# mfkiwl/conan-slam

Measured on AMD Instinct MI355X. Metric: ekf_update_steps_per_sec, higher is better.
Workload: dtype f32

## Files before the change

conan_slam_amd/_capi.py:

```python
from __future__ import annotations

import ctypes as C
import os
import re

_HERE = os.path.dirname(os.path.abspath(__file__))
LIB_PATH = os.path.join(_HERE, "lib", "libcslam_hip.so")
HEADER_PATH = os.path.join(_HERE, "..", "include", "cslam.h")

OK, ERR_BAD_ARG, ERR_CAPACITY, ERR_HIP, ERR_NO_DEVICE, ERR_ALLOC = 0, 1, 2, 3, 4, 5
FACTOR_OK, FACTOR_FALLBACK, FACTOR_ZEROED, FACTOR_SKIPPED, FACTOR_BAD_IDF, FACTOR_INTERNAL = 0, 1, 2, 4, 8, 16
FACTOR_HEADING_SKIPPED = 32
F32, F64 = 0, 1
Q_LOWER_CHOL_GAIN, Q_PREDICT_NM4, Q_REF_EXACT, Q_TEXTBOOK = 1, 2, 3, 0
STAGE_GATHER, STAGE_FACTOR, STAGE_GAIN, STAGE_DOWNDATE, N_STAGES = 0, 1, 2, 3, 4
STAGE_NAMES = ["gather", "factor", "gain", "downdate"]


class CslamError(RuntimeError):
    def __init__(self, code: int, msg: str):
        super().__init__(f"cslam status {code}: {msg}")
        self.code = code


BATCH_MC_SYMBOLS = ("cslam_ekf_batch_predict_each", "cslam_ekf_batch_get_poses")

LANDMARK_SYMBOLS = ("cslam_ekf_get_landmarks", "cslam_ekf_batch_get_landmarks")
_PROTOTYPES = {
    "cslam_ekf_get_landmarks": [C.c_void_p, C.c_int, C.c_int, C.c_void_p, C.c_void_p, C.c_void_p],
    "cslam_ekf_batch_get_landmarks": [C.c_void_p, C.c_int, C.c_int, C.c_void_p, C.c_void_p, C.c_void_p],
    "cslam_ekf_rows_launches": [C.c_void_p, C.POINTER(C.c_longlong)],
    "cslam_ekf_pgemm_split": [C.c_void_p, C.POINTER(C.c_int), C.POINTER(C.c_int)],
    "cslam_ekf_batch_pgemm_split": [C.c_void_p, C.POINTER(C.c_int), C.POINTER(C.c_int)],
    "cslam_sim_batch_create": [C.c_void_p, C.c_int, C.c_int, C.POINTER(C.c_longlong), C.c_int, C.POINTER(C.c_void_p)],
    "cslam_sim_batch_destroy": [C.c_void_p],
    "cslam_sim_batch_scan": [C.c_void_p, C.c_void_p, C.c_double, C.c_void_p, C.c_longlong, C.POINTER(C.c_int),
                             C.POINTER(C.c_int), C.POINTER(C.c_int)],
    "cslam_sim_batch_get_scan": [C.c_void_p, C.c_int, C.c_void_p, C.c_void_p, C.c_void_p, C.c_void_p],
    "cslam_sim_batch_get_table": [C.c_void_p, C.c_void_p],
    "cslam_sim_batch_set_table": [C.c_void_p, C.c_void_p],
    "cslam_ekf_batch_update_scan": [C.c_void_p, C.c_void_p, C.c_void_p],
    "cslam_ekf_batch_augment_scan": [C.c_void_p, C.c_void_p, C.c_void_p],
    "cslam_pf_best_particle": [C.c_void_p, C.c_int, C.POINTER(C.c_int)] + [C.c_void_p] * 5,
    "cslam_pf_estimate": [C.c_void_p, C.POINTER(C.c_double), C.POINTER(C.c_double)] + [C.c_void_p] * 4,
    "cslam_pf_get_all_features": [C.c_void_p, C.c_void_p],
    "cslam_pf_best_particle_sharded": [C.c_void_p, C.c_void_p, C.c_int, C.POINTER(C.c_longlong)] + [C.c_void_p] * 5,
    "cslam_pf_estimate_sharded": [C.c_void_p, C.c_void_p, C.POINTER(C.c_double), C.POINTER(C.c_double)]
                                 + [C.c_void_p] * 4,
}
PF_ESTIMATE_SYMBOLS = tuple(k for k in _PROTOTYPES if k.startswith("cslam_pf_"))
PF_PICK_MAX, PF_PICK_MIN = 0, 1
SIM_BATCH_SYMBOLS = tuple(k for k in _PROTOTYPES if "sim_batch" in k or k.endswith("_scan"))

SCORE_FIELD_NAMES = ("POSE_N", "POSE_BAD", "POSE_IN", "POSE_ERR2", "POSE_EPHI2", "POSE_NEES",
                     "LM_N", "LM_BAD", "LM_IN", "LM_ERR2", "LM_NEES")
(SCORE_POSE_N, SCORE_POSE_BAD, SCORE_POSE_IN, SCORE_POSE_ERR2, SCORE_POSE_EPHI2, SCORE_POSE_NEES,
 SCORE_LM_N, SCORE_LM_BAD, SCORE_LM_IN, SCORE_LM_ERR2, SCORE_LM_NEES) = range(len(SCORE_FIELD_NAMES))
SCORE_FIELDS = len(SCORE_FIELD_NAMES)
_PROTOTYPES.update({
    "cslam_ekf_batch_score_reset": [C.c_void_p, C.c_int, C.c_double, C.c_double],
    "cslam_ekf_batch_score_set_truth": [C.c_void_p, C.c_void_p, C.c_int],
    "cslam_ekf_batch_score": [C.c_void_p, C.c_void_p],
    "cslam_ekf_batch_score_scan": [C.c_void_p, C.c_void_p, C.c_void_p],
    "cslam_ekf_batch_get_scores": [C.c_void_p, C.c_void_p, C.c_void_p, C.c_int, C.POINTER(C.c_int),
# ... 181 lines not shown
```

conan_slam_amd/csrc/cslam_ekf.hip:

```cpp
#include <hip/hip_runtime.h>

#include <algorithm>
#include <atomic>
#include <cfloat>
#include <cmath>
#include <cstdint>
#include <cstdlib>
#include <new>
#include <string>
#include <thread>
#include <vector>

#include "cslam_common.hpp"
#include "device_owners.hpp"
#include "ekf_kernels.hpp"
#include "ekf_kernels_fast.hpp"
#include "ekf_assoc_deferred_kernels.hpp"
#include "ekf_augment_kernels.hpp"
#include "ekf_counted_kernels.hpp"
#include "ekf_landmark_kernels.hpp"
#include "ekf_lookahead.hpp"
#include "ekf_options.hpp"
#include "ekf_pending_store.hpp"
#include "ekf_pgemm_limbs.hpp"
#include "ekf_pgemm_tiles.hpp"
#include "ekf_pose_kernels.hpp"
#define CSLAM_SCORE_SINGLE_ONLY
#include "ekf_score_kernels.hpp"
#include "ekf_staging.hpp"
#include "host_linalg.hpp"
#include "pf_host_parts.hpp"

namespace cslam
{
__global__ void ekf_la_signal_kernel(unsigned* signal, unsigned add)
{
    if (threadIdx.x == 0)
    {
        atomicAdd(signal, add);
    }
}
__device__ __forceinline__ bool la_wide_snapshot(const LaSnapJob& j)
{
    if (j.Z == nullptr || blockIdx.x + 1 != gridDim.x)
    {
        return false;
    }
    for (int i = threadIdx.x; i < 3 * j.m; i += 128)
    {
        if (i < 2 * j.m)
        {
            j.Z_out[i] = j.Z[i];
        }
        else
        {
            j.idf_out[i - 2 * j.m] = j.idf[i - 2 * j.m];
        }
    }
    return true;
}
__global__ void __launch_bounds__(128) ekf_la_wide_f32(LaWideArgs a)
{
    if (la_wide_snapshot(a.snap))
    {
        return;
    }
    ekf_la_wide_body<1, 0>(a);
}
__global__ void __launch_bounds__(128) ekf_la_wide_f32_k64(LaWideArgs a)
{
    if (la_wide_snapshot(a.snap))
    {
        return;
    }
    ekf_la_wide_body<1, 64>(a);
}

__global__ void __launch_bounds__(128) ekf_la_wide_f32_k64m(LaWideArgs a, float* WT)
{
    if (la_wide_snapshot(a.snap))
    {
        return;
    }
    ekf_la_wide_body<1, 64, 1>(a, WT);
}

__global__ void __launch_bounds__(256) ekf_la_blocks_mirror_kernel(LaPrepArgs<float> a, LaMirrorArgs mi)
{
    ekf_la_blocks_mirror_body(a, mi);
}
}

using namespace cslam;

namespace
{

std::atomic<int>& g_engines = ::cslam::live_engines();

constexpr size_t kLdsBudget    = 150 * 1024;

struct EkfBase
{
    explicit EkfBase(const EkfOptions& o) : opt(o) {}
    virtual ~EkfBase() {}
    const EkfOptions opt;
    int         dtype    = CSLAM_F32;
    int         device   = 0;
    int         quirks   = CSLAM_Q_REF_EXACT;
    int         nmax     = 0;
    int         ncap     = 0;
    int         ldp      = 0;
    int         n        = 3;
    int         sync_mode = 1;
    int         pgemm_wgs     = 0;
    int         split_whole = 0, split_strips = 0;
    Stream      stream_own, stream_b_own, stream_f_own;
    hipStream_t stream   = nullptr;
    hipStream_t stream_b = nullptr;
    long long   la_windows = 0;
    long long   stage_launches = 0;
    long long   rows_launches = 0;
    long long   augment_launches = 0;

    virtual int init()                                                                        = 0;
    virtual int set_state(const void* X, int n, const void* P, int ldp)                        = 0;
    virtual int get_state(void* X, void* P, int ldp)                                           = 0;
    virtual int get_x(void* X, int cap)                                                        = 0;
    virtual int get_landmarks(int first, int count, void* x, void* pll, void* pvl)             = 0;
    virtual int trace(double* tr)                                                              = 0;
    virtual int get_pose(void* x, void* pvv)                                                   = 0;
    virtual int score_reset(int series_capacity, double gate_pose, double gate_lm)             = 0;
    virtual int score_set_truth(const double* lm_true, int count)                              = 0;
    virtual int score(const double* xv_true, int with_map)                                     = 0;
    virtual int get_scores(double* totals, float* series, double* track, int capacity_records, int* records,
                           long long* calls)                                                   = 0;
    virtual int predict(double v, double swa, const void* Q, double wb, double dt)             = 0;
    virtual int update(const void* Z, int m, const void* R, const int* idf, int batch, bool on_device) = 0;
    virtual int augment(const void* Z, int q, const void* R)                                   = 0;
    virtual int augment_device(const void* dZ, int q, const void* R)                           = 0;
    virtual int observe_heading(double phi, int use)                                           = 0;
    virtual int associate(const void* Z, int m, const void* R, double g1, double g2, int* idf_out, int* kind) = 0;
    virtual int update_counted(const void* dZ, int m_cap, const void* R, const int* d_idf, const int* d_count,
                               int batch)                                                      = 0;
    virtual int associate_deferred(const void* Z, int m, const void* R, double g1, double g2, int* idf_out, int* kind,
                                   int* counts)                                                = 0;
    virtual int associate_deferred_async(const void* Z, int m, const void* R, double g1, double g2) = 0;
    virtual int association_wait(int* idf_out, int* kind, int* counts)                         = 0;
    virtual int association_device_ptrs(const void** dZF, const int** d_idf, const void** dZN,
                                        const int** d_counts)                                  = 0;
    virtual int factor_status(int* flags, int clear)                                           = 0;
    virtual int set_profiling(int on)                                                          = 0;
    virtual int get_stage_times(double* ms, int* launches)                                     = 0;
    virtual int debug_last_update(void* PHT, void* S, void* G, void* W1, void* V, int* k)      = 0;
    virtual int set_deferred(int max_cols)                                                     = 0;
// ... 1639 lines not shown
                return rc;
            }
        }
        CSLAM_HIP_TRY(hipStreamSynchronize(stream));
        return CSLAM_OK;
    }


    struct LaUpd
    {
        const T*       dZ;
        const int*     dIdf;
        int            m;
        T              R[4];
        PredictArgs<T> pp;
    };
    struct FactorOut
    {
        DevBuf<T>   S, G, Gt, V, t, U, M, sub, xloc;
        DevBuf<int> idloc;
    };
    struct LaSet
    {
        Event          ev_fb;
        Event          ev_raw;
        FactorOut      fo[2];
        DevBuf<T>      XL, PvL, PH, PvLb, Dbb;
        DevBuf<T>      Y;
        DevBuf<LaModel<T>> model;
        DevBuf<unsigned>   done;
        DevBuf<long long>  stamps;
        DevBuf<int>        idf_keep;
        DevBuf<T>          z_keep;
    };
    struct LaHeld
    {
        bool       valid = false;
        bool       k64   = false;
        unsigned   grid  = 0;
        LaWideArgs wa;
        float*     wt = nullptr;
    };
    LaHeld      la_held;
    LaUpd       la_q[2];
    int         la_n = 0;
    LaSet       la;
    bool        la_ready = false;
    hipStream_t stream_f = nullptr;
    DevBuf<T>   la_WR;
    int         la_kpad  = 0;
    int         la_cus = 0;
    unsigned    la_target = 0;
    unsigned    la_seq    = 0;
    unsigned    la_sig_add = 0;
    DevBuf<float> la_WT;
    int           la_wt_rows     = 0;
    const T *dbgS = nullptr, *dbgGt = nullptr, *dbgV = nullptr;

    int la_ensure(int kp_cols)
    {
        constexpr int KM = 2 * kLaMaxObs;
        if (!la_ready)
        {
            int lo = 0, hi = 0;
            CSLAM_HIP_TRY(hipDeviceGetStreamPriorityRange(&lo, &hi));
            Stream sf;
            LaSet  nl;
            int    rc = sf.create_with_priority(hipStreamNonBlocking, hi);
            if (rc || (rc = nl.ev_fb.create(hipEventDisableTiming)) || (rc = nl.ev_raw.create(hipEventDisableTiming)))
            {
                return rc;
            }
            CSLAM_HIP_TRY(hipFuncSetAttribute(reinterpret_cast<const void*>(&ekf_la_chain_kernel<T, 32>),
                                              hipFuncAttributeMaxDynamicSharedMemorySize, (int)la_chain_lds<T>(32)));
            CSLAM_HIP_TRY(hipFuncSetAttribute(reinterpret_cast<const void*>(&ekf_la_chain_kernel<T, 64>),
                                              hipFuncAttributeMaxDynamicSharedMemorySize, (int)la_chain_lds<T>(64)));
            CSLAM_TRY(nl.done.alloc_zeroed_blocking(768));
            for (FactorOut& f : nl.fo)
            {
                const size_t kk = (size_t)KM * (KM + 1);
                if ((rc = f.S.alloc(kk)) || (rc = f.G.alloc(kk)) || (rc = f.Gt.alloc(kk)) || (rc = f.V.alloc(KM)) ||
                    (rc = f.t.alloc(KM)) || (rc = f.U.alloc(KM)) || (rc = f.M.alloc((size_t)3 * KM)) ||
                    (rc = f.sub.alloc((size_t)(3 + KM) * KM)) || (rc = f.xloc.alloc(3 + KM)) ||
                    (rc = f.idloc.alloc(kLaMaxObs)))
                {
                    return rc;
                }
            }
            if ((rc = nl.XL.alloc((size_t)2 * KM)) || (rc = nl.PvL.alloc((size_t)2 * KM * 3)) ||
                (rc = nl.PH.alloc((size_t)KM * KM)) || (rc = nl.PvLb.alloc((size_t)KM * 3)) ||
                (rc = nl.Dbb.alloc((size_t)KM * KM)) || (rc = nl.Y.alloc((size_t)KM * KM)) ||
                (rc = nl.model.alloc(2)) || (rc = nl.idf_keep.alloc(kLaMaxObs)) ||
                (rc = nl.z_keep.alloc(2 * kLaMaxObs)) ||
                (opt.la_stamps && (rc = nl.stamps.alloc_zeroed_blocking(32))))
            {
                return rc;
            }
            stream_f_own = std::move(sf);
            stream_f     = stream_f_own.get();
            la           = std::move(nl);
            la_cus       = 1;
            la_target    = 0;
            la_seq       = 0;
            la_ready     = true;
        }
        if (kp_cols > la_kpad)
        {
            CSLAM_HIP_TRY(hipStreamSynchronize(stream));
            CSLAM_HIP_TRY(hipStreamSynchronize(stream_f));
// ... 21 lines not shown
    {
        const int k = 2 * m;
        const bool on = opt.lookahead > 0 || (opt.lookahead < 0 && sizeof(T) == 4 && n >= 7000 && g_engines.load() == 1);
        return on && !sync_mode && !opt.pipeline && prof.mode != 1 && k > 16 && k <= 2 * kLaMaxObs && opt.gather_corr_wide &&
               opt.fuse_predict && (sizeof(T) == 4 || opt.fuse_f64) && defer_max >= k + (la_n ? 2 * la_q[0].m : k) &&
               pend.wcap >= k + (la_n ? 2 * la_q[0].m : k) && seq.count == 0 && pend.hd_cols[0] == 0 && pend.hd_cols[1] == 0 && n > 3 &&
               kp_call_limit == 0;
    }

    int la_launch_held_wide(const LaSnapJob* job)
    {
        if (!la_held.valid)
        {
            return CSLAM_OK;
        }
        if constexpr (std::is_same<T, float>::value)
        {
            int rc = use_device();
            if (rc)
            {
                return rc;
            }
            if (g_engines.load() > 1)
            {
                CSLAM_HIP_TRY(hipStreamWaitEvent(stream, la.ev_fb.get(), 0));
            }
            LaWideArgs& wa = la_held.wa;
            unsigned    g  = la_held.grid;
            if (job != nullptr)
            {
                wa.snap = *job;
                g += 1;
            }
            if (la_held.k64 && la_held.wt != nullptr)
            {
                hipLaunchKernelGGL(ekf_la_wide_f32_k64m, dim3(g), dim3(128), 0, stream, wa, la_held.wt);
            }
            else if (la_held.k64)
            {
                hipLaunchKernelGGL(ekf_la_wide_f32_k64, dim3(g), dim3(128), 0, stream, wa);
            }
            else
            {
                hipLaunchKernelGGL(ekf_la_wide_f32, dim3(g), dim3(128), 0, stream, wa);
            }
            CSLAM_HIP_TRY(hipGetLastError());
        }
        la_held.valid = false;
        return CSLAM_OK;
    }

    int la_enqueue(const T* dZ, const int* dIdf, int m, const T* R, bool on_device)
    {
        if (on_device && la_n == 0)
        {
            int rc = la_held.valid ? ensure_m(m) : CSLAM_OK;
            if (rc)
            {
                return rc;
            }
            if constexpr (std::is_same<T, float>::value)
            {
                if (la_held.valid)
                {
                    unsigned char* ds = ring.dev_slot(ring.take_slot());
                    LaSnapJob      job;
                    job.Z       = dZ;
// ... 264 lines not shown

    int la_launch_window(bool may_hold = false)
    {
        if (la_n == 0)
        {
            return CSLAM_OK;
        }
        const int   nu = la_n;
        const LaUpd ua = la_q[0], ub = la_q[nu - 1];
        const int   ka = 2 * ua.m, kb = nu == 2 ? 2 * ub.m : 0;
        la_n = 0;
        const PredictArgs<T> held = pp;
        int rc = use_device();
        if (rc)
        {
            return rc;
        }
        if (pend.kp > 256 && (rc = flush()))
        {
            return rc;
        }
        if ((rc = ensure_k(2 * kLaMaxObs)) || (rc = ensure_w(ka + kb)) || (rc = la_ensure(pend.kp)))
        {
            return rc;
        }
        if (opt.lower && (rc = ensure_tile_list(round_up(n, kTile) / kTile)))
        {
            return rc;
        }
        const bool safe = g_engines.load() > 1;
        const unsigned n_blocks = (unsigned)(3 + ka + 2 * kb);
        const bool hold = may_hold && opt.la_hold_wide && opt.la_fused && !safe && nu == 2 && std::is_same<T, float>::value &&
                 !la.stamps.get();
        auto launch_chain = [&]() -> int {
            const LaChainArgs<T> ch = la_chain_args(ua, ub, nu, hold, la_target + n_blocks, ++la_seq);
            if (std::max(ka, kb) <= 32)
            {
                hipLaunchKernelGGL((ekf_la_chain_kernel<T, 32>), dim3(1), dim3(256), la_chain_lds<T>(32), stream_f, ch);
            }
            else
            {
                hipLaunchKernelGGL((ekf_la_chain_kernel<T, 64>), dim3(1), dim3(256), la_chain_lds<T>(64), stream_f, ch);
            }
            CSLAM_HIP_TRY(hipGetLastError());
            CSLAM_HIP_TRY(hipEventRecord(la.ev_fb.get(), stream_f));
            return CSLAM_OK;
        };
        if (!safe && (rc = launch_chain()))
        {
            return rc;
        }
        bool use_mirror = false;
        if constexpr (std::is_same<T, float>::value)
        {
            use_mirror = opt.la_mirror &&
                         (pend.kp == 0 || (pend.mirror_covers(pend.kp, n) && pend.kp <= 128 && pend.kp % 4 == 0));
        }
        const int  k8f       = round_up(pend.kp, 8);
        const bool pg_signal = !opt.la_wg_signal && !safe && pend.kp > 0 && seq.count == 0 && sizeof(T) == 4 && k8f <= 128 &&
                               opt.lower && ldp < 32768 && !limbs_take(k8f) && stream_b == stream &&
                               pend.hd_cols[pend.wcur] == 0;
        if constexpr (std::is_same<T, float>::value)
        {
            if (use_mirror)
            {
                hipLaunchKernelGGL(ekf_la_blocks_mirror_kernel, dim3(n_blocks), dim3(256), 0, stream,
                                   la_prep_args(ua, ub, nu, hold, pg_signal), la_mirror_args(ua, ub, nu, hold));
            }
// ... 6 lines not shown
        }
        CSLAM_HIP_TRY(hipGetLastError());
        if (safe)
        {
            CSLAM_HIP_TRY(hipEventRecord(la.ev_raw.get(), stream));
            CSLAM_HIP_TRY(hipStreamWaitEvent(stream_f, la.ev_raw.get(), 0));
            if ((rc = launch_chain()))
            {
                return rc;
            }
        }
        la_target += n_blocks;
        la_sig_add = pg_signal ? n_blocks : 0u;
        rc         = flush();
        if (la_sig_add != 0)
        {
            const unsigned add = la_sig_add;
            la_sig_add         = 0;
            hipLaunchKernelGGL(ekf_la_signal_kernel, dim3(1), dim3(64), 0, stream, la.done.get(), add);
        }
        if (rc)
        {
            return rc;
        }
        bool fused = false;
        if constexpr (std::is_same<T, float>::value)
        {
            if (opt.la_fused)
            {
                fused = true;
                la_held.wa  = la_wide_args(ua, ub, nu, hold);
                la_held.k64 = opt.la_k64 && ua.m == 32 && ub.m == 32;
                la_held.wt = (opt.la_mirror && la_held.k64 && pend.kp == 0) ? la_WT.get() : nullptr;
                pend.mirror_written(la_held.wt ? ka + kb : 0, n);
                la_held.grid  = (unsigned)(round_up(n, kTile) / 32);
                la_held.valid = true;
                if (!hold && (rc = la_launch_held_wide(nullptr)))
                {
                    return rc;
                }
                last_slot = nullptr;
                last_k    = 0;
                pend.appended(ka + kb);
                sub_valid = false;
            }
        }
        if (!fused && ((rc = la_wide(ua, la.fo[0], la.ev_fb.get())) || (nu == 2 && (rc = la_wide(ub, la.fo[1], nullptr)))))
        {
            return rc;
        }
        pp = held;
        la_windows++;
        return (la.stamps.get() && la_windows == 300) ? la_report_stamps() : CSLAM_OK;
    }

    int la_report_stamps()
    {
        long long h[32];
        CSLAM_HIP_TRY(hipStreamSynchronize(stream));
        CSLAM_HIP_TRY(hipMemcpy(h, la.stamps.get(), sizeof(h), hipMemcpyDeviceToHost));
        fprintf(stderr, "[cslam la wide stamps, 10 ns ticks] ids+columns issue:%lld poll+DMA wait:%lld pht_a:%lld gain_a:%lld store+share W1_a:%lld pht_b+corr:%lld share+G_b:%lld gain_b:%lld store_b:%lld\n",
                h[17] - h[16], h[18] - h[17], h[19] - h[18], h[20] - h[19], h[21] - h[20], h[22] - h[21], h[23] - h[22],
                h[24] - h[23], h[25] - h[24]);
        fprintf(stderr, "[cslam la stamps, cycles] load+observe:%lld sums:%lld symmetrise:%lld cholesky:%lld (first half %lld) inverse:%lld outputs:%lld total:%lld\n",
                h[6] - h[0], h[7] - h[6], h[1] - h[7], h[2] - h[1], h[5] ? h[5] - h[1] : 0, h[3] - h[2], h[4] - h[3], h[4] - h[0]);
        return CSLAM_OK;
// ... 983 lines not shown
{
    CSLAM_NEED(h);
    if (!whole_tiles || !strips)
    {
        return fail(CSLAM_ERR_BAD_ARG, "pgemm_split: null");
    }
    *whole_tiles = B(h)->split_whole;
    *strips      = B(h)->split_strips;
    return CSLAM_OK;
}

int cslam_ekf_lookahead_windows(cslam_ekf_t h, long long* windows)
{
    CSLAM_NEED(h);
    if (!windows)
    {
        return fail(CSLAM_ERR_BAD_ARG, "lookahead_windows: null");
    }
    *windows = B(h)->la_windows;
    return CSLAM_OK;
}

int cslam_ekf_rows_launches(cslam_ekf_t h, long long* launches)
{
    CSLAM_NEED(h);
    if (!launches)
    {
        return fail(CSLAM_ERR_BAD_ARG, "rows_launches: null");
    }
    *launches = B(h)->rows_launches;
    return CSLAM_OK;
}

int cslam_ekf_stage_launches(cslam_ekf_t h, long long* launches)
{
    CSLAM_NEED(h);
    if (!launches)
    {
        return fail(CSLAM_ERR_BAD_ARG, "stage_launches: null");
    }
    *launches = B(h)->stage_launches;
    return CSLAM_OK;
}

int cslam_ekf_get_streams(cslam_ekf_t h, void** chain_stream, void** pgemm_stream)
{
    CSLAM_NEED(h);
    if (chain_stream)
    {
        *chain_stream = reinterpret_cast<void*>(B(h)->stream);
    }
    if (pgemm_stream)
    {
        *pgemm_stream = reinterpret_cast<void*>(B(h)->stream_b);
    }
    return CSLAM_OK;
}

int cslam_ekf_run_many(cslam_ekf_t* handles, int count, int steps, const double* v, const double* swa, const void* Q,
                       double wb, double dt, const void* const* dZ, const int* const* d_idf, int m, const void* R,
                       int batch)
{
    if (!handles || count < 0 || steps < 0 || m < 0 || !R || !Q || (steps > 0 && (!v || !swa)) || (m > 0 && (!dZ || !d_idf)))
    {
        return fail(CSLAM_ERR_BAD_ARG, "run_many: bad arguments");
    }
// ... 99 lines not shown
```

conan_slam_amd/csrc/ekf_lookahead.hpp:

```cpp
#pragma once

#include <hip/hip_runtime.h>

#include "ekf_kernels.hpp"
#include "ekf_kernels_fast.hpp"

namespace cslam
{

constexpr int kLaMaxObs = 32;

__device__ inline int la_row(const int* __restrict__ idf, int s, int n)
{
    return 3 + 2 * clamp_idf(idf[s >> 1], n) - 2 + (s & 1);
}

template <typename T>
struct LaRowsArgs
{
    const T* X;
    const T* Pv;
    int      ldp, n;
    const int* idf_a;
    int        ra;
// ... 903 lines not shown
        mo.g02 = s_g[0];
        mo.g12 = s_g[1];
    }
    if (tid < 3)
    {
        mo.pose[tid] = xl[tid];
    }
    if (tid < 9)
    {
        mo.pvv[tid] = s_pvv[tid];
    }
    for (int e = tid; e < mb * 10; e += 256)
    {
        mo.coef[e] = coef[e];
    }
}

constexpr int kFlagLaTimeout = 16;

template <typename T>
struct LaChainArgs
{
    FactorArgs<T>   fa, fb;
    T *             du_a, *du_b;
    LaCarryArgs<T>  ca;
    int             nu;
    const unsigned* done;
    unsigned        target;
    unsigned long long timeout;
    unsigned*       chain_done;
    unsigned        seq;
};

template <typename T, int K>
__device__ __forceinline__ void ekf_la_chain_body(const LaChainArgs<T>& a)
{
    extern __shared__ __align__(16) unsigned char la_chain_smem[];
    if (threadIdx.x < 64)
    {
        const unsigned long long t0 = __builtin_amdgcn_s_memrealtime();
        while (true)
        {
            unsigned c = threadIdx.x < 16
                             ? __hip_atomic_load(a.done + 16 * threadIdx.x, __ATOMIC_RELAXED, __HIP_MEMORY_SCOPE_AGENT)
                             : 0u;
            c += __shfl_xor(c, 1);
            c += __shfl_xor(c, 2);
            c += __shfl_xor(c, 4);
            c += __shfl_xor(c, 8);
            c = __shfl(c, 0);
            if ((int)(c - a.target) >= 0)
            {
                break;
            }
            __builtin_amdgcn_s_sleep(32);
            if (__builtin_amdgcn_s_memrealtime() - t0 > a.timeout)
            {
                if (threadIdx.x == 0)
                {
                    atomicOr(&a.fa.flags[0], kFlagLaTimeout);
                }
                break;
            }
        }
    }
    __syncthreads();
    __builtin_amdgcn_fence(__ATOMIC_ACQUIRE, "agent");
    if constexpr (std::is_same<T, float>::value)
    {
        ekf_factor_mfma_f32_body<K>(a.fa, a.du_a);
    }
    else
    {
        ekf_factor_mfma_f64_body<K>(a.fa, a.du_a);
    }
    if (a.nu == 2)
    {
        __builtin_amdgcn_fence(__ATOMIC_RELEASE, "workgroup");
        __syncthreads();
        __builtin_amdgcn_fence(__ATOMIC_ACQUIRE, "workgroup");
        ekf_la_carry_body<T>(a.ca, la_chain_smem);
        __builtin_amdgcn_fence(__ATOMIC_RELEASE, "workgroup");
        __syncthreads();
        __builtin_amdgcn_fence(__ATOMIC_ACQUIRE, "workgroup");
        if constexpr (std::is_same<T, float>::value)
        {
            ekf_factor_mfma_f32_body<K>(a.fb, a.du_b);
        }
        else
        {
            ekf_factor_mfma_f64_body<K>(a.fb, a.du_b);
        }
    }
    __builtin_amdgcn_fence(__ATOMIC_RELEASE, "agent");
    __syncthreads();
    if (threadIdx.x < 32)
    {
        __hip_atomic_store(a.chain_done + 16 * threadIdx.x, a.seq, __ATOMIC_RELAXED, __HIP_MEMORY_SCOPE_AGENT);
    }
}

template <typename T, int K>
__global__ void __launch_bounds__(256) ekf_la_chain_kernel(LaChainArgs<T> a)
{
    ekf_la_chain_body<T, K>(a);
}

struct LaSnapJob
{
    const float* Z;
    const int*   idf;
    float*       Z_out;
    int*         idf_out;
    int          m;
};

struct LaWideArgs
{
    const float* P;
    int          ldp, n, lower;
    float*       X;
    float*       Pv;
    int          nu;
    const int *  idf_a, *idf_b;
    int          ma, mb;
    int          valid_a, valid_b, w_a, w_b;
// ... 620 lines not shown
```

conan_slam_amd/csrc/ekf_options.hpp:

```cpp
#pragma once

#include <algorithm>
#include <cstdlib>
#include <cstring>

namespace cslam
{
inline int env_int(const char* name, int dflt) { const char* s = getenv(name); return s ? atoi(s) : dflt; }
inline int env_flag(const char* name, int dflt) { const char* s = getenv(name); return s ? (atoi(s) ? 1 : 0) : dflt; }
constexpr int kPgemmTailMax = 1 << 20;
inline int env_pgemm_tail(int dflt) { return std::max(-1, std::min(kPgemmTailMax, env_int("CSLAM_PGEMM_TAIL", dflt))); }

struct EkfOptions
{
    int fuse_predict = 1;
    int fuse_f64     = 1;
    int seq_defer    = 1;
    int lower = 1;
    int pipeline    = 0;
    int pgemm_spare = 16;
    int gather_corr_wide = 1;
    int lookahead    = -1;
    int la_hold_wide = 1;
    int la_k64       = 1;
    int la_wg_signal = 0;
    int la_mirror    = 1;
    int la_fused     = 1;
    int la_stamps    = 0;
    int pgemm_limbs = 0;
    int limbs_kmin  = 65;
    int xcd_queues = 0;
    int psym_nt    = -1;
    int pgemm_tail = -1;
    int f64_kcm = 16;
    int f64_cb  = 0;

    static EkfOptions from_env()
    {
        EkfOptions o;
        o.fuse_predict     = env_int("CSLAM_FUSE_PREDICT", o.fuse_predict);
        o.fuse_f64         = env_flag("CSLAM_FUSE_F64", o.fuse_f64);
        o.seq_defer        = env_int("CSLAM_SEQ_DEFER", o.seq_defer);
        const char* sv     = getenv("CSLAM_STORAGE");
        o.lower            = (sv && !strcmp(sv, "full")) ? 0 : 1;
        o.pipeline         = env_flag("CSLAM_PIPELINE", o.pipeline);
        o.pgemm_spare      = std::max(0, env_int("CSLAM_PGEMM_SPARE", o.pgemm_spare));
        o.gather_corr_wide = env_flag("CSLAM_GATHER_WIDE", o.gather_corr_wide);
        const int la       = env_int("CSLAM_LOOKAHEAD", o.lookahead);
        o.lookahead        = la > 0 ? 1 : (la < 0 ? -1 : 0);
        o.la_hold_wide     = env_flag("CSLAM_LA_HOLD_WIDE", o.la_hold_wide);
        o.la_k64           = env_flag("CSLAM_LA_K64", o.la_k64);
        o.la_wg_signal     = env_flag("CSLAM_LA_WG_SIGNAL", o.la_wg_signal);
        o.la_mirror        = env_flag("CSLAM_LA_MIRROR", o.la_mirror);
        o.la_fused         = env_flag("CSLAM_LA_FUSED", o.la_fused);
        o.la_stamps        = getenv("CSLAM_LA_STAMPS") ? 1 : 0;
        const int limbs    = env_int("CSLAM_PGEMM_LIMBS", o.pgemm_limbs);
        o.pgemm_limbs      = (limbs == 6 || limbs == 9) ? limbs : 0;
        const int kmin     = env_int("CSLAM_LIMBS_KMIN", o.limbs_kmin);
        o.limbs_kmin       = kmin < 0 ? o.limbs_kmin : std::max(57, kmin);
        o.xcd_queues       = env_flag("CSLAM_XCD_QUEUES", o.xcd_queues);
        o.psym_nt          = env_flag("CSLAM_PSYM_NT", o.psym_nt);
        o.pgemm_tail       = env_pgemm_tail(o.pgemm_tail);
        o.f64_kcm          = std::max(4, std::min(64, (env_int("CSLAM_F64_KCM", o.f64_kcm) + 3) / 4 * 4));
        if (getenv("CSLAM_F64_CB"))
        {
            o.f64_cb = env_int("CSLAM_F64_CB", 0) == 2 ? 2 : 4;
        }
        return o;
    }
};

struct EkfBatchOptions
{
    int wg_signal  = 0;
    int wide_pairs = 2;
    int la_k64     = 1;
    int stamps     = 0;
    int pgemm_tail = -1;

    static EkfBatchOptions from_env()
    {
        EkfBatchOptions o;
        o.wg_signal  = env_flag("CSLAM_BATCH_WG_SIGNAL", o.wg_signal);
        o.wide_pairs = env_int("CSLAM_BATCH_WIDE_PAIRS", o.wide_pairs) == 1 ? 1 : 2;
        o.la_k64     = env_flag("CSLAM_LA_K64", o.la_k64);
        o.stamps     = getenv("CSLAM_BATCH_STAMPS") ? 1 : 0;
        o.pgemm_tail = env_pgemm_tail(o.pgemm_tail);
// ... 6 lines not shown
```

conan_slam_amd/ekf.py:

```python
from __future__ import annotations

import ctypes as C

import numpy as np

from . import _capi
from ._capi import (F32, F64, Q_REF_EXACT, Q_TEXTBOOK, check)


def _vp(a: np.ndarray):
    return a.ctypes.data_as(C.c_void_p)


class EKF:
    def __init__(self, max_landmarks: int, dtype=np.float32, device: int = -1, quirks: int = Q_REF_EXACT,
                 sync_mode: bool = True):
        self.dtype = np.dtype(dtype)
        if self.dtype not in (np.dtype(np.float32), np.dtype(np.float64)):
            raise ValueError("dtype must be float32 or float64")
        self._L = _capi.lib()
        self._h = C.c_void_p(None)
        code = F32 if self.dtype == np.float32 else F64
        check(self._L.cslam_ekf_create(C.c_int(max_landmarks), C.c_int(code), C.c_int(device), C.c_int(quirks),
                                       C.byref(self._h)))
# ... 71 lines not shown
    P = property(get_p)

    def trace(self) -> float:
        t = C.c_double(0.0)
        check(self._L.cslam_ekf_trace(self._h, C.byref(t)))
        return t.value

    def synchronize(self):
        check(self._L.cslam_ekf_synchronize(self._h))

    def pgemm_split(self):
        w, s = C.c_int(0), C.c_int(0)
        check(self._L.cslam_ekf_pgemm_split(self._h, C.byref(w), C.byref(s)))
        return w.value, s.value

    def lookahead_windows(self) -> int:
        w = C.c_longlong(0)
        check(self._L.cslam_ekf_lookahead_windows(self._h, C.byref(w)))
        return w.value

    def streams(self):
        a, b = C.c_void_p(None), C.c_void_p(None)
        check(self._L.cslam_ekf_get_streams(self._h, C.byref(a), C.byref(b)))
        return a.value or 0, b.value or 0

    def stage_launches(self) -> int:
        w = C.c_longlong(0)
        check(self._L.cslam_ekf_stage_launches(self._h, C.byref(w)))
        return w.value

    def rows_launches(self) -> int:
        w = C.c_longlong(0)
        check(self._L.cslam_ekf_rows_launches(self._h, C.byref(w)))
        return w.value

    def landmarks(self, first: int = 1, count: int = None):
        if count is None:
            count = max((self.n - 3) // 2 - first + 1, 0)
        x = np.empty((count, 2), dtype=self.dtype)
        pll = np.empty((count, 4), dtype=self.dtype)
        pvl = np.empty((count, 6), dtype=self.dtype)
        check(self._L.cslam_ekf_get_landmarks(self._h, int(first), int(count), _vp(x), _vp(pll), _vp(pvl)))
        return x, pll.reshape(count, 2, 2).transpose(0, 2, 1).copy(), pvl.reshape(count, 2, 3).transpose(0, 2, 1).copy()

    def pose(self):
        x = np.empty(3, dtype=self.dtype)
        pv = np.empty(9, dtype=self.dtype)
        check(self._L.cslam_ekf_get_pose(self._h, _vp(x), _vp(pv)))
        return x, pv.reshape(3, 3).T.copy()

    def factor_status(self, clear: bool = False) -> int:
        f = C.c_int(0)
        check(self._L.cslam_ekf_factor_status(self._h, C.byref(f), C.c_int(1 if clear else 0)))
        return f.value

    def score_reset(self, series_capacity: int = 0, gate_pose: float = 0.0, gate_lm: float = 0.0):
        check(self._L.cslam_ekf_score_reset(self._h, C.c_int(int(series_capacity)), C.c_double(float(gate_pose)),
                                            C.c_double(float(gate_lm))))

    def score_set_truth(self, lm_true):
        t = np.ascontiguousarray(np.asarray(lm_true, dtype=np.float64).reshape(-1, 2))
        check(self._L.cslam_ekf_score_set_truth(self._h, _vp(t) if t.size else None, C.c_int(t.shape[0])))

    def score(self, xv_true, with_map: bool = True):
        x = np.ascontiguousarray(np.asarray(xv_true, dtype=np.float64).reshape(3))
        check(self._L.cslam_ekf_score(self._h, _vp(x), C.c_int(1 if with_map else 0)))
# ... 380 lines not shown
```

include/cslam.h:

```cpp
#ifndef CSLAM_H
#define CSLAM_H

#ifdef __cplusplus
extern "C" {
#endif

#define CSLAM_VERSION 100

#define CSLAM_OK 0
#define CSLAM_ERR_BAD_ARG 1
#define CSLAM_ERR_CAPACITY 2
#define CSLAM_ERR_HIP 3
#define CSLAM_ERR_NO_DEVICE 4
#define CSLAM_ERR_ALLOC 5
#define CSLAM_FACTOR_OK 0
#define CSLAM_FACTOR_FALLBACK 1
#define CSLAM_FACTOR_ZEROED 2
#define CSLAM_FACTOR_SKIPPED 4
#define CSLAM_FACTOR_INTERNAL 16
#define CSLAM_FACTOR_BAD_IDF 8
#define CSLAM_FACTOR_HEADING_SKIPPED 32
#define CSLAM_FACTOR_COUNT_CLAMPED 64

#define CSLAM_F32 0
// ... 42 lines not shown

int cslam_ekf_augment_device(cslam_ekf_t h, const void* dZ, int q, const void* R);

int cslam_ekf_augment_launches(cslam_ekf_t h, long long* launches);

int cslam_ekf_observe_heading(cslam_ekf_t h, double phi, int use_heading);

int cslam_ekf_associate(cslam_ekf_t h, const void* Z, int m, const void* R, double gate1, double gate2, int* idf_out,
                        int* kind_out);

int cslam_ekf_associate_deferred(cslam_ekf_t h, const void* Z, int m, const void* R, double gate1, double gate2,
                                 int* idf_out, int* kind_out, int* counts_out );

int cslam_ekf_association_device_ptrs(cslam_ekf_t h, const void** dZF, const int** d_idf, const void** dZN,
                                      const int** d_counts);

int cslam_ekf_associate_deferred_async(cslam_ekf_t h, const void* Z, int m, const void* R, double gate1, double gate2);

int cslam_ekf_association_wait(cslam_ekf_t h, int* idf_out, int* kind_out, int* counts_out );

int cslam_ekf_update_counted(cslam_ekf_t h, const void* dZ, int m_cap, const void* R, const int* d_idf, const int* d_count,
                             int batch);

int cslam_ekf_set_deferred(cslam_ekf_t h, int max_pending_columns);
int cslam_ekf_flush(cslam_ekf_t h);

int cslam_ekf_get_streams(cslam_ekf_t h, void** chain_stream, void** pgemm_stream);

int cslam_ekf_lookahead_windows(cslam_ekf_t h, long long* windows);

int cslam_ekf_stage_launches(cslam_ekf_t h, long long* launches);

int cslam_ekf_rows_launches(cslam_ekf_t h, long long* launches);

int cslam_ekf_set_pgemm_workgroups(cslam_ekf_t h, int workgroups);

int cslam_ekf_pgemm_split(cslam_ekf_t h, int* whole_tiles, int* strips);

int cslam_ekf_run_many(cslam_ekf_t* handles, int count, int steps, const double* v, const double* swa, const void* Q,
                       double wb, double dt, const void* const* dZ, const int* const* d_idf, int m, const void* R,
                       int batch);

typedef struct cslam_ekf_batch* cslam_ekf_batch_t;
int cslam_ekf_batch_create(int instances, int n_landmarks, int device, int quirks, cslam_ekf_batch_t* out);
int cslam_ekf_batch_destroy(cslam_ekf_batch_t h);
int cslam_ekf_batch_set_state(cslam_ekf_batch_t h, int instance, const float* X, int n, const float* P, int ldp);
int cslam_ekf_batch_get_state(cslam_ekf_batch_t h, int instance, float* X, float* P, int ldp);
int cslam_ekf_batch_run(cslam_ekf_batch_t h, int steps, const double* v, const double* swa, const float* Q, double wb,
                        double dt, const float* const* dZ, const int* const* d_idf, int m, const float* R);
int cslam_ekf_batch_flush(cslam_ekf_batch_t h);
int cslam_ekf_batch_synchronize(cslam_ekf_batch_t h);
int cslam_ekf_batch_trace(cslam_ekf_batch_t h, double* traces );
int cslam_ekf_batch_factor_status(cslam_ekf_batch_t h, int* flags );
int cslam_ekf_batch_info(cslam_ekf_batch_t h, int* instances, int* n, long long* windows);
int cslam_ekf_batch_set_profiling(cslam_ekf_batch_t h, int every);
int cslam_ekf_batch_get_pgemm_time(cslam_ekf_batch_t h, double* ms_sum, int* launches);
int cslam_ekf_batch_pgemm_split(cslam_ekf_batch_t h, int* whole_tiles, int* strips);

int cslam_ekf_batch_create_capacity(int instances, int max_landmarks, int n_landmarks, int device, int quirks,
                                    cslam_ekf_batch_t* out);
int cslam_ekf_batch_predict(cslam_ekf_batch_t h, double v, double swa, const float* Q, double wb, double dt);
int cslam_ekf_batch_predict_each(cslam_ekf_batch_t h, const double* v, const double* swa, const float* Q, double wb,
                                 double dt);
int cslam_ekf_batch_get_poses(cslam_ekf_batch_t h, float* x, float* pvv);
int cslam_ekf_batch_get_landmarks(cslam_ekf_batch_t h, int first, int count, float* x, float* pll, float* pvl);

// ... 167 lines not shown
```

Baseline: 14200.

## Publish swizzled gain operand images from chain kernel for wide lookahead kernel

The factor chain kernel gains a post-hook that rewrites Gt and Y into transposed, XOR-swizzled 64x64 images in global memory. A new wide kernel then DMAs these images straight into LDS with buffer-load-to-LDS and feeds them to MFMA without per-block transposes. The aim is to move the operand relayout out of every wide workgroup into a single chain-side pass. The cost is extra global buffers plus an extra store pass in the serial chain kernel. It is on by default, with an env flag to disable it and a launch counter added.

```diff
diff --git a/conan_slam_amd/_capi.py b/conan_slam_amd/_capi.py
--- a/conan_slam_amd/_capi.py
+++ b/conan_slam_amd/_capi.py
@@ -30,6 +30,7 @@
     "cslam_ekf_get_landmarks": [C.c_void_p, C.c_int, C.c_int, C.c_void_p, C.c_void_p, C.c_void_p],
     "cslam_ekf_batch_get_landmarks": [C.c_void_p, C.c_int, C.c_int, C.c_void_p, C.c_void_p, C.c_void_p],
     "cslam_ekf_rows_launches": [C.c_void_p, C.POINTER(C.c_longlong)],
+    "cslam_ekf_wide_ops_launches": [C.c_void_p, C.POINTER(C.c_longlong)],
     "cslam_ekf_pgemm_split": [C.c_void_p, C.POINTER(C.c_int), C.POINTER(C.c_int)],
     "cslam_ekf_batch_pgemm_split": [C.c_void_p, C.POINTER(C.c_int), C.POINTER(C.c_int)],
     "cslam_sim_batch_create": [C.c_void_p, C.c_int, C.c_int, C.POINTER(C.c_longlong), C.c_int, C.POINTER(C.c_void_p)],
diff --git a/conan_slam_amd/csrc/cslam_ekf.hip b/conan_slam_amd/csrc/cslam_ekf.hip
--- a/conan_slam_amd/csrc/cslam_ekf.hip
+++ b/conan_slam_amd/csrc/cslam_ekf.hip
@@ -20,6 +20,7 @@
 #include "ekf_counted_kernels.hpp"
 #include "ekf_landmark_kernels.hpp"
 #include "ekf_lookahead.hpp"
+#include "ekf_la_wide_ops.hpp"
 #include "ekf_options.hpp"
 #include "ekf_pending_store.hpp"
 #include "ekf_pgemm_limbs.hpp"
@@ -83,6 +84,19 @@
         return;
     }
     ekf_la_wide_body<1, 64, 1>(a, WT);
+}
+
+__global__ void __launch_bounds__(128) ekf_la_wide_f32_k64m_ops(LaWideArgs a, LaOpsImages im, float* WT)
+{
+    if (la_wide_snapshot(a.snap))
+    {
+        return;
+    }
+    ekf_la_wide_ops_body(a, im, WT);
+}
+__global__ void __launch_bounds__(256) ekf_la_chain_ops_kernel(LaChainArgs<float> a, LaOpsPublish pub)
+{
+    ekf_la_chain_body<float, 64>(a, pub);
 }
 
 __global__ void __launch_bounds__(256) ekf_la_blocks_mirror_kernel(LaPrepArgs<float> a, LaMirrorArgs mi)
@@ -121,6 +135,7 @@
     long long   la_windows = 0;
     long long   stage_launches = 0;
     long long   rows_launches = 0;
+    long long   wide_ops_launches = 0;
     long long   augment_launches = 0;
 
     virtual int init()                                                                        = 0;
@@ -1826,6 +1841,7 @@
         DevBuf<long long>  stamps;
         DevBuf<int>        idf_keep;
         DevBuf<T>          z_keep;
+        DevBuf<float>      ops_G[2], ops_Y;
     };
     struct LaHeld
     {
@@ -1834,6 +1850,7 @@
         unsigned   grid  = 0;
         LaWideArgs wa;
         float*     wt = nullptr;
+        bool       ops = false;
     };
     LaHeld      la_held;
     LaUpd       la_q[2];
@@ -1869,6 +1886,16 @@
                                               hipFuncAttributeMaxDynamicSharedMemorySize, (int)la_chain_lds<T>(32)));
             CSLAM_HIP_TRY(hipFuncSetAttribute(reinterpret_cast<const void*>(&ekf_la_chain_kernel<T, 64>),
                                               hipFuncAttributeMaxDynamicSharedMemorySize, (int)la_chain_lds<T>(64)));
+            if constexpr (std::is_same<T, float>::value)
+            {
+                CSLAM_HIP_TRY(hipFuncSetAttribute(reinterpret_cast<const void*>(&ekf_la_chain_ops_kernel),
+                                                  hipFuncAttributeMaxDynamicSharedMemorySize, (int)la_chain_lds<T>(64)));
+                if ((rc = nl.ops_G[0].alloc((size_t)KM * KM)) || (rc = nl.ops_G[1].alloc((size_t)KM * KM)) ||
+                    (rc = nl.ops_Y.alloc((size_t)KM * KM)))
+                {
+                    return rc;
+                }
+            }
             CSLAM_TRY(nl.done.alloc_zeroed_blocking(768));
             for (FactorOut& f : nl.fo)
             {
@@ -1956,7 +1983,13 @@
                 wa.snap = *job;
                 g += 1;
             }
-            if (la_held.k64 && la_held.wt != nullptr)
+            if (la_held.k64 && la_held.wt != nullptr && la_held.ops)
+            {
+                const LaOpsImages im{la.ops_G[0].get(), la.ops_G[1].get(), la.ops_Y.get()};
+                hipLaunchKernelGGL(ekf_la_wide_f32_k64m_ops, dim3(g), dim3(128), 0, stream, wa, im, la_held.wt);
+                wide_ops_launches++;
+            }
+            else if (la_held.k64 && la_held.wt != nullptr)
             {
                 hipLaunchKernelGGL(ekf_la_wide_f32_k64m, dim3(g), dim3(128), 0, stream, wa, la_held.wt);
             }
@@ -2287,8 +2320,22 @@
         const unsigned n_blocks = (unsigned)(3 + ka + 2 * kb);
         const bool hold = may_hold && opt.la_hold_wide && opt.la_fused && !safe && nu == 2 && std::is_same<T, float>::value &&
                  !la.stamps.get();
+        const bool chain_ops = opt.la_wide_ops && opt.la_fused && opt.la_k64 && opt.la_mirror && !safe &&
+                               std::is_same<T, float>::value && ua.m == 32 && ub.m == 32;
         auto launch_chain = [&]() -> int {
             const LaChainArgs<T> ch = la_chain_args(ua, ub, nu, hold, la_target + n_blocks, ++la_seq);
+            if constexpr (std::is_same<T, float>::value)
+            {
+                if (chain_ops)
+                {
+                    const LaOpsPublish pub{la.fo[0].Gt.get(),  la.fo[1].Gt.get(),  la.Y.get(),
+                                           la.ops_G[0].get(), la.ops_G[1].get(), la.ops_Y.get(), nu};
+                    hipLaunchKernelGGL(ekf_la_chain_ops_kernel, dim3(1), dim3(256), la_chain_lds<T>(64), stream_f, ch, pub);
+                    CSLAM_HIP_TRY(hipGetLastError());
+                    CSLAM_HIP_TRY(hipEventRecord(la.ev_fb.get(), stream_f));
+                    return CSLAM_OK;
+                }
+            }
             if (std::max(ka, kb) <= 32)
             {
                 hipLaunchKernelGGL((ekf_la_chain_kernel<T, 32>), dim3(1), dim3(256), la_chain_lds<T>(32), stream_f, ch);
@@ -2361,6 +2408,7 @@
                 la_held.wa  = la_wide_args(ua, ub, nu, hold);
                 la_held.k64 = opt.la_k64 && ua.m == 32 && ub.m == 32;
                 la_held.wt = (opt.la_mirror && la_held.k64 && pend.kp == 0) ? la_WT.get() : nullptr;
+                la_held.ops = chain_ops && la_held.wt != nullptr;
                 pend.mirror_written(la_held.wt ? ka + kb : 0, n);
                 la_held.grid  = (unsigned)(round_up(n, kTile) / 32);
                 la_held.valid = true;
@@ -3410,6 +3458,17 @@
     return CSLAM_OK;
 }
 
+int cslam_ekf_wide_ops_launches(cslam_ekf_t h, long long* launches)
+{
+    CSLAM_NEED(h);
+    if (!launches)
+    {
+        return fail(CSLAM_ERR_BAD_ARG, "wide_ops_launches: null");
+    }
+    *launches = B(h)->wide_ops_launches;
+    return CSLAM_OK;
+}
+
 int cslam_ekf_stage_launches(cslam_ekf_t h, long long* launches)
 {
     CSLAM_NEED(h);
diff --git a/conan_slam_amd/csrc/ekf_la_wide_ops.hpp b/conan_slam_amd/csrc/ekf_la_wide_ops.hpp
--- /dev/null
+++ b/conan_slam_amd/csrc/ekf_la_wide_ops.hpp
@@ -0,0 +1,407 @@
+#pragma once
+
+#include "ekf_lookahead.hpp"
+
+namespace cslam
+{
+
+__host__ __device__ __forceinline__ int la_ops_index(int i, int j)
+{
+    return j * 64 + ((((i >> 2) ^ (j & 15)) << 2) | (i & 3));
+}
+
+struct LaOpsPublish
+{
+    const float *Gt_a, *Gt_b, *Y_b;
+    float *      Ga, *Gb, *Yb;
+    int          nu;
+    __device__ __forceinline__ void operator()() const
+    {
+        __builtin_amdgcn_fence(__ATOMIC_RELEASE, "workgroup");
+        __syncthreads();
+        __builtin_amdgcn_fence(__ATOMIC_ACQUIRE, "workgroup");
+        const int    i0 = 4 * (threadIdx.x >> 4), j0 = 4 * (threadIdx.x & 15);
+        const float* src[3] = {Gt_a, Gt_b, Y_b};
+        float*       dst[3] = {Ga, Gb, Yb};
+        const int    cnt    = nu == 2 ? 3 : 1;
+        float4       v[3][4];
+#pragma unroll
+        for (int s = 0; s < 3; s++)
+        {
+#pragma unroll
+            for (int r = 0; r < 4; r++)
+            {
+                v[s][r] = s < cnt ? *reinterpret_cast<const float4*>(src[s] + (i0 + r) * 64 + j0) : make_float4(0.f, 0.f, 0.f, 0.f);
+            }
+        }
+#pragma unroll
+        for (int s = 0; s < 3; s++)
+        {
+            if (s < cnt)
+            {
+                float* d = dst[s];
+                *reinterpret_cast<float4*>(d + la_ops_index(i0, j0))     = make_float4(v[s][0].x, v[s][1].x, v[s][2].x, v[s][3].x);
+                *reinterpret_cast<float4*>(d + la_ops_index(i0, j0 + 1)) = make_float4(v[s][0].y, v[s][1].y, v[s][2].y, v[s][3].y);
+                *reinterpret_cast<float4*>(d + la_ops_index(i0, j0 + 2)) = make_float4(v[s][0].z, v[s][1].z, v[s][2].z, v[s][3].z);
+                *reinterpret_cast<float4*>(d + la_ops_index(i0, j0 + 3)) = make_float4(v[s][0].w, v[s][1].w, v[s][2].w, v[s][3].w);
+            }
+        }
+    }
+};
+
+struct LaOpsImages
+{
+    const float *Ga, *Gb, *Yb;
+};
+
+__device__ __forceinline__ void ekf_la_wide_ops_body(const LaWideArgs& a, const LaOpsImages& im, float* wt)
+{
+    constexpr int K   = 64;
+    constexpr int kXs = 20;
+    __shared__ __attribute__((aligned(16))) float s_G[2][4 * 1024];
+    __shared__ __attribute__((aligned(16))) float s_Y[4 * 1024];
+    __shared__ __attribute__((aligned(16))) float s_model[2][512];
+    __shared__ __attribute__((aligned(16))) float s_u[2][256];
+    __shared__ __attribute__((aligned(16))) float s_M[2][256];
+    __shared__ int   s_fx[2][kLaMaxObs];
+    __shared__ float s_sum[4][32];
+    const int tid = threadIdx.x, wv =__builtin_amdgcn_readfirstlane(tid >> 6), lane = tid & 63, lj = lane & 31, lh = lane >> 5;
+    const int row0 = blockIdx.x * 32;
+    const int row  = row0 + lj;
+    const int rowc = row < a.n ? row : a.n - 1;
+    int       stamp_i = 0;
+    auto      stamp   = [&]() {
+        if (a.stamps != nullptr && blockIdx.x == (gridDim.x >> 1) && tid == 0)
+        {
+            a.stamps[stamp_i++] = (long long)__builtin_amdgcn_s_memrealtime();
+        }
+    };
+    stamp();
+    const int id_a = lane < a.ma ? a.idf_a[lane] : 1;
+    const int id_b = (a.nu == 2 && lane < a.mb) ? a.idf_b[lane] : 1;
+    float pv0 = a.Pv[(size_t)0 * a.ldp + rowc], pv1 = a.Pv[(size_t)1 * a.ldp + rowc], pv2 = a.Pv[(size_t)2 * a.ldp + rowc];
+    float x   = a.X[rowc];
+    if (tid < kLaMaxObs)
+    {
+        s_fx[0][tid] = 3 + 2 * clamp_idf(id_a, a.n) - 2;
+        s_fx[1][tid] = 3 + 2 * clamp_idf(id_b, a.n) - 2;
+    }
+    __syncthreads();
+    float pcol[2][16];
+    {
+        int fxv[2][8];
+#pragma unroll
+        for (int ub = 0; ub < 2; ub++)
+        {
+#pragma unroll
+            for (int i = 0; i < 8; i++)
+            {
+                const int o = (32 * wv + (2 * i & 3) + 8 * (2 * i >> 2) + 4 * lh) >> 1;
+                fxv[ub][i]  = s_fx[ub][o];
+            }
+        }
+#pragma unroll
+        for (int ub = 0; ub < 2; ub++)
+        {
+#pragma unroll
+            for (int i = 0; i < 8; i++)
+            {
+                const bool in = ub == 0 || a.nu == 2;
+                const int  fx = in ? fxv[ub][i] : 3;
+                const float va = p_sym<float>(a.P, a.ldp, rowc, fx, a.lower);
+                const float vb = p_sym<float>(a.P, a.ldp, rowc, fx + 1, a.lower);
+                pcol[ub][2 * i]     = in ? va : 0.f;
+                pcol[ub][2 * i + 1] = in ? vb : 0.f;
+            }
+        }
+    }
+    stamp();
+    if (tid == 0)
+    {
+        const unsigned long long t0   = __builtin_amdgcn_s_memrealtime();
+        const unsigned*          word = a.chain_done + 16 * (blockIdx.x & 31u);
+        while ((int)(__hip_atomic_load(word, __ATOMIC_RELAXED, __HIP_MEMORY_SCOPE_AGENT) - a.seq) < 0)
+        {
+            __builtin_amdgcn_s_sleep(8);
+            if (__builtin_amdgcn_s_memrealtime() - t0 > a.timeout)
+            {
+                atomicOr(&a.flags[0], kFlagLaTimeout);
+                break;
+            }
+        }
+    }
+    __syncthreads();
+    __builtin_amdgcn_fence(__ATOMIC_ACQUIRE, "agent");
+    typedef __attribute__((address_space(3))) void* lptr_t;
+    auto dma = [&](const float* src, int count, float* dst) {
+        const __amdgpu_buffer_rsrc_t rs =
+            __builtin_amdgcn_make_buffer_rsrc(const_cast<float*>(src), 0, (unsigned)(count * 4), 0x00020000);
+        const int pieces = (count + 255) / 256;
+        int       it     = (int)(blockIdx.x & 15u);
+        it               = it < pieces ? it : 0;
+        for (int j = 0; j < pieces; j++, it = (it + 1 < pieces) ? it + 1 : 0)
+        {
+            if ((j % 2) == wv)
+            {
+                __builtin_amdgcn_raw_ptr_buffer_load_lds(rs, (lptr_t)(dst + it * 256), 16, (unsigned)(lane * 16),
+                                                         (unsigned)(it * 1024), 0, 0);
+            }
+        }
+    };
+    dma(im.Ga, K * K, s_G[0]);
+    dma(reinterpret_cast<const float*>(a.model_a), 336, s_model[0]);
+    dma(a.u_a, K, s_u[0]);
+    dma(a.M_a, 3 * K, s_M[0]);
+    if (a.nu == 2)
+    {
+        dma(im.Yb, K * K, s_Y);
+        dma(reinterpret_cast<const float*>(a.model_b), 336, s_model[1]);
+        dma(a.u_b, K, s_u[1]);
+        dma(a.M_b, 3 * K, s_M[1]);
+    }
+    __builtin_amdgcn_s_waitcnt(0x0F70);
+    __syncthreads();
+    stamp();
+    const int sw0 = (32 * wv + lj) * 64 + ((lh ^ (lj & 15)) << 2);
+    float* xch = s_G[1];
+    float  own[16];
+    float  full[32];
+    auto share = [&]() {
+#pragma unroll
+        for (int g = 0; g < 4; g++)
+        {
+            *reinterpret_cast<float4*>(xch + (wv * 64 + lane) * kXs + 4 * g) =
+                make_float4(own[4 * g], own[4 * g + 1], own[4 * g + 2], own[4 * g + 3]);
+        }
+        __syncthreads();
+#pragma unroll
+        for (int t = 0; t < 2; t++)
+        {
+#pragma unroll
+            for (int g = 0; g < 4; g++)
+            {
+                const float4 v = *reinterpret_cast<const float4*>(xch + (t * 64 + lane) * kXs + 4 * g);
+                full[t * 16 + 4 * g]     = v.x;
+                full[t * 16 + 4 * g + 1] = v.y;
+                full[t * 16 + 4 * g + 2] = v.z;
+                full[t * 16 + 4 * g + 3] = v.w;
+            }
+        }
+    };
+    auto build_own = [&](auto UB, const float* sub) {
+        constexpr int ub = decltype(UB)::value;
+#pragma unroll
+        for (int i = 0; i < 8; i++)
+        {
+            const int    r = 2 * i;
+            const int    q = 32 * wv + (r & 3) + 8 * (r >> 2) + 4 * lh;
+            const float* c = &s_model[ub][14 + (q >> 1) * 10];
+            float        v0, v1;
+            la_pht_pair<float>(c, pv0, pv1, pv2, pcol[ub][2 * i], pcol[ub][2 * i + 1], &v0, &v1);
+            const bool in = row < a.n;
+            if (row < 3 && in)
+            {
+                v0 = sub[row * K + q];
+                v1 = sub[row * K + q + 1];
+            }
+            own[r]     = in ? v0 : 0.f;
+            own[r + 1] = in ? v1 : 0.f;
+        }
+    };
+    f32x16 w1;
+    auto   gain = [&](auto UB) {
+        constexpr int ub = decltype(UB)::value;
+        const float*  Gs = s_G[ub];
+        const float*  v0 = wv == 0 ? s_u[ub] : s_M[ub] + K;
+        const float*  v1 = wv == 0 ? s_M[ub] : s_M[ub] + 2 * K;
+        f32x16        ac0 = f32x16{0}, ac1 = f32x16{0};
+        float         sa = 0.f, sb = 0.f;
+        float4        g[8], e0[8], e1[8];
+#pragma unroll
+        for (int i = 0; i < 8; i++)
+        {
+            const int q0 = 32 * (i >> 2) + 8 * (i & 3) + 4 * lh;
+            g[i]  = *reinterpret_cast<const float4*>(Gs + (sw0 ^ ((8 * (i >> 2) + 2 * (i & 3)) << 2)));
+            e0[i] = *reinterpret_cast<const float4*>(v0 + q0);
+            e1[i] = *reinterpret_cast<const float4*>(v1 + q0);
+        }
+#pragma unroll
+        for (int i = 0; i < 32; i++)
+        {
+            const float b  = full[i];
+            const float gv = (i & 3) == 0 ? g[i >> 2].x : (i & 3) == 1 ? g[i >> 2].y : (i & 3) == 2 ? g[i >> 2].z : g[i >> 2].w;
+            const float ea = (i & 3) == 0 ? e0[i >> 2].x : (i & 3) == 1 ? e0[i >> 2].y : (i & 3) == 2 ? e0[i >> 2].z : e0[i >> 2].w;
+            const float eb = (i & 3) == 0 ? e1[i >> 2].x : (i & 3) == 1 ? e1[i >> 2].y : (i & 3) == 2 ? e1[i >> 2].z : e1[i >> 2].w;
+            if (i & 1)
+            {
+                ac1 = __builtin_amdgcn_mfma_f32_32x32x2f32(gv, b, ac1, 0, 0, 0);
+            }
+            else
+            {
+                ac0 = __builtin_amdgcn_mfma_f32_32x32x2f32(gv, b, ac0, 0, 0, 0);
+            }
+            sa += b * ea;
+            sb += b * eb;
+        }
+#pragma unroll
+        for (int r = 0; r < 16; r++)
+        {
+            w1[r] = ac0[r] + ac1[r];
+        }
+        sa += __shfl_xor(sa, 32);
+        sb += __shfl_xor(sb, 32);
+        if (lh == 0)
+        {
+            s_sum[2 * wv][lj]     = sa;
+            s_sum[2 * wv + 1][lj] = sb;
+        }
+    };
+    auto store_w1 = [&](float* W, bool last) {
+#pragma unroll
+        for (int r = 0; r < 16; r++)
+        {
+            const int c = la_q_of(wv, r, lh);
+            if (row < 3)
+            {
+                if (last)
+                {
+                    a.wv_out[(size_t)row * K + c] = w1[r];
+                }
+                W[(size_t)c * a.ldw + row] = 0.f;
+            }
+            else
+            {
+                W[(size_t)c * a.ldw + row] = w1[r];
+            }
+        }
+    };
+    auto store_wt = [&](int q0) {
+        float* dst = wt + (size_t)row * 128 + q0 + 32 * wv + 4 * lh;
+#pragma unroll
+        for (int g = 0; g < 4; g++)
+        {
+            const float4 v = make_float4(w1[4 * g], w1[4 * g + 1], w1[4 * g + 2], w1[4 * g + 3]);
+            *reinterpret_cast<float4*>(dst + 8 * g) = (row < 3) ? make_float4(0.f, 0.f, 0.f, 0.f) : v;
+        }
+    };
+    using U0 = std::integral_constant<int, 0>;
+    using U1 = std::integral_constant<int, 1>;
+
+    if (a.valid_a && row >= 3 && row - 3 < a.w_a)
+    {
+        float o0, o1, o2;
+        predict_stripe_col<float>(s_model[0][0], s_model[0][1], pv0, pv1, pv2, &o0, &o1, &o2);
+        pv0 = o0, pv1 = o1, pv2 = o2;
+    }
+    build_own(U0{}, a.sub_a);
+    share();
+    stamp();
+    gain(U0{});
+    stamp();
+    store_w1(a.W1a, a.nu == 1);
+    store_wt(0);
+    const float* pred_last = s_model[0];
+    if (a.nu == 2)
+    {
+        __syncthreads();
+#pragma unroll
+        for (int r = 0; r < 16; r++)
+        {
+            own[r] = (row >= 3) ? w1[r] : 0.f;
+        }
+        share();
+        const float xs = s_sum[0][lj], xm0 = s_sum[1][lj], xm1 = s_sum[2][lj], xm2 = s_sum[3][lj];
+        if (row >= 3)
+        {
+            x += xs;
+            pv0 -= xm0, pv1 -= xm1, pv2 -= xm2;
+        }
+        stamp();
+        if (a.valid_b && row >= 3 && row - 3 < a.w_b)
+        {
+            float o0, o1, o2;
+            predict_stripe_col<float>(s_model[1][0], s_model[1][1], pv0, pv1, pv2, &o0, &o1, &o2);
+            pv0 = o0, pv1 = o1, pv2 = o2;
+        }
+        build_own(U1{}, a.sub_b);
+        {
+            f32x16 c0 = f32x16{0}, c1 = f32x16{0};
+            float4 y[8];
+#pragma unroll
+            for (int i = 0; i < 8; i++)
+            {
+                y[i] = *reinterpret_cast<const float4*>(s_Y + (sw0 ^ ((8 * (i >> 2) + 2 * (i & 3)) << 2)));
+            }
+#pragma unroll
+            for (int i = 0; i < 32; i++)
+            {
+                const float yv = (i & 3) == 0 ? y[i >> 2].x : (i & 3) == 1 ? y[i >> 2].y : (i & 3) == 2 ? y[i >> 2].z : y[i >> 2].w;
+                if (i & 1)
+                {
+                    c1 = __builtin_amdgcn_mfma_f32_32x32x2f32(yv, full[i], c1, 0, 0, 0);
+                }
+                else
+                {
+                    c0 = __builtin_amdgcn_mfma_f32_32x32x2f32(yv, full[i], c0, 0, 0, 0);
+                }
+            }
+            if (row >= 3)
+            {
+#pragma unroll
+                for (int r = 0; r < 16; r++)
+                {
+                    own[r] -= c0[r] + c1[r];
+                }
+            }
+        }
+        stamp();
+        __syncthreads();
+        dma(im.Gb, K * K, s_G[1]);
+        xch = s_G[0];
+        share();
+        __builtin_amdgcn_s_waitcnt(0x0F70);
+        __syncthreads();
+        stamp();
+        gain(U1{});
+        stamp();
+        store_w1(a.W1b, true);
+        store_wt(64);
+        pred_last = s_model[1];
+    }
+    __syncthreads();
+    stamp();
+    if (wv == 0 && lh == 0 && row < a.n)
+    {
+        const float xs = s_sum[0][lj], xm0 = s_sum[1][lj], xm1 = s_sum[2][lj], xm2 = s_sum[3][lj];
+        if (row >= 3)
+        {
+            a.X[row]                      = x + xs;
+            a.Pv[(size_t)0 * a.ldp + row] = pv0 - xm0;
+            a.Pv[(size_t)1 * a.ldp + row] = pv1 - xm1;
+            a.Pv[(size_t)2 * a.ldp + row] = pv2 - xm2;
+        }
+        else
+        {
+            const int   r     = row;
+            const float av[3] = {pred_last[5 + r], pred_last[5 + r + 3], pred_last[5 + r + 6]};
+            const float dv[3] = {xm0, xm1, xm2};
+            a.X[r]            = pred_last[2 + r] + xs;
+#pragma unroll
+            for (int c = 0; c < 3; c++)
+            {
+                if (c == r)
+                {
+                    a.Pv[(size_t)c * a.ldp + r] = av[c] - dv[c];
+                }
+                else if (c < r)
+                {
+                    const float bcr             = pred_last[5 + c + 3 * r];
+                    a.Pv[(size_t)c * a.ldp + r] = av[c] - dv[c];
+                    a.Pv[(size_t)r * a.ldp + c] = bcr - dv[c];
+                }
+            }
+        }
+    }
+}
+
+}
diff --git a/conan_slam_amd/csrc/ekf_lookahead.hpp b/conan_slam_amd/csrc/ekf_lookahead.hpp
--- a/conan_slam_amd/csrc/ekf_lookahead.hpp
+++ b/conan_slam_amd/csrc/ekf_lookahead.hpp
@@ -959,8 +959,13 @@
     unsigned        seq;
 };
 
-template <typename T, int K>
-__device__ __forceinline__ void ekf_la_chain_body(const LaChainArgs<T>& a)
+struct LaChainNoPost
+{
+    __device__ __forceinline__ void operator()() const {}
+};
+
+template <typename T, int K, typename Post = LaChainNoPost>
+__device__ __forceinline__ void ekf_la_chain_body(const LaChainArgs<T>& a, const Post& post = Post{})
 {
     extern __shared__ __align__(16) unsigned char la_chain_smem[];
     if (threadIdx.x < 64)
@@ -1019,6 +1024,7 @@
             ekf_factor_mfma_f64_body<K>(a.fb, a.du_b);
         }
     }
+    post();
     __builtin_amdgcn_fence(__ATOMIC_RELEASE, "agent");
     __syncthreads();
     if (threadIdx.x < 32)
diff --git a/conan_slam_amd/csrc/ekf_options.hpp b/conan_slam_amd/csrc/ekf_options.hpp
--- a/conan_slam_amd/csrc/ekf_options.hpp
+++ b/conan_slam_amd/csrc/ekf_options.hpp
@@ -26,6 +26,7 @@
     int la_wg_signal = 0;
     int la_mirror    = 1;
     int la_fused     = 1;
+    int la_wide_ops  = 1;
     int la_stamps    = 0;
     int pgemm_limbs = 0;
     int limbs_kmin  = 65;
@@ -53,6 +54,7 @@
         o.la_wg_signal     = env_flag("CSLAM_LA_WG_SIGNAL", o.la_wg_signal);
         o.la_mirror        = env_flag("CSLAM_LA_MIRROR", o.la_mirror);
         o.la_fused         = env_flag("CSLAM_LA_FUSED", o.la_fused);
+        o.la_wide_ops      = env_flag("CSLAM_LA_WIDE_OPS", o.la_wide_ops);
         o.la_stamps        = getenv("CSLAM_LA_STAMPS") ? 1 : 0;
         const int limbs    = env_int("CSLAM_PGEMM_LIMBS", o.pgemm_limbs);
         o.pgemm_limbs      = (limbs == 6 || limbs == 9) ? limbs : 0;
diff --git a/conan_slam_amd/ekf.py b/conan_slam_amd/ekf.py
--- a/conan_slam_amd/ekf.py
+++ b/conan_slam_amd/ekf.py
@@ -127,6 +127,11 @@
     def rows_launches(self) -> int:
         w = C.c_longlong(0)
         check(self._L.cslam_ekf_rows_launches(self._h, C.byref(w)))
+        return w.value
+
+    def wide_ops_launches(self) -> int:
+        w = C.c_longlong(0)
+        check(self._L.cslam_ekf_wide_ops_launches(self._h, C.byref(w)))
         return w.value
 
     def landmarks(self, first: int = 1, count: int = None):
diff --git a/include/cslam.h b/include/cslam.h
--- a/include/cslam.h
+++ b/include/cslam.h
@@ -98,6 +98,8 @@
 int cslam_ekf_stage_launches(cslam_ekf_t h, long long* launches);
 
 int cslam_ekf_rows_launches(cslam_ekf_t h, long long* launches);
+
+int cslam_ekf_wide_ops_launches(cslam_ekf_t h, long long* launches);
 
 int cslam_ekf_set_pgemm_workgroups(cslam_ekf_t h, int workgroups);
 
```

Result: no change. 14160, median of 2 (-0.3%).
